# KKKSQJ/DeepLearning

Hardware: NVIDIA H100
Metric: images/sec (ResNet-50 training step) (higher is better)
Workload: dtype bf16

## Files before the change

deeplearning_b200/csrc/abi_conv.cu:

```cuda
#include <string.h>
#include "../../include/b200cls.h"
#include "conv_gemm.cuh"
#include "conv1x1_stream.cuh"
#include "conv_tap64.cuh"
#include "host_utils.h"
#include "wgrad_gemm.cuh"

using namespace b200;

namespace {

constexpr uint32_t kFwdDescLbo = 16, kFwdDescSbo = 1024;
constexpr uint32_t kWgDescLbo = 8192, kWgDescSbo = 1024, kWgDescKstep = 2048;

struct Box3 {
  int b1, b2, b3;
};

Box3 choose_box(long long d1, long long d2, long long d3, int P) {
  Box3 best{P, 1, 1};
  double best_cost = -1;
  for (int b1 = 1; b1 <= P; b1 <<= 1) {
    for (int b2 = 1; b1 * b2 <= P; b2 <<= 1) {
      const int b3 = P / (b1 * b2);
// ... 101 lines not shown
  for (int q = 0; q < 4; ++q) o1[q] = o2[q] = o3[q] = 0;
  if (bx.b3 >= 4) {
    *qb = Box3{bx.b1, bx.b2, bx.b3 / 4};
    for (int q = 0; q < 4; ++q) o3[q] = q * (bx.b3 / 4);
  } else if (bx.b3 == 2) {
    *qb = Box3{bx.b1, bx.b2 / 2, 1};
    if (bx.b2 >= 2) {
      for (int q = 0; q < 4; ++q) {
        o2[q] = (q & 1) * (bx.b2 / 2);
        o3[q] = q >> 1;
      }
    } else {
      *qb = Box3{bx.b1 / 2, 1, 1};
      for (int q = 0; q < 4; ++q) {
        o1[q] = (q & 1) * (bx.b1 / 2);
        o3[q] = q >> 1;
      }
    }
  } else if (bx.b2 >= 4) {
    *qb = Box3{bx.b1, bx.b2 / 4, 1};
    for (int q = 0; q < 4; ++q) o2[q] = q * (bx.b2 / 4);
  } else if (bx.b2 == 2) {
    *qb = Box3{bx.b1 / 2, 1, 1};
    for (int q = 0; q < 4; ++q) {
      o1[q] = (q & 1) * (bx.b1 / 2);
      o2[q] = q >> 1;
    }
  } else {
    *qb = Box3{bx.b1 / 4, 1, 1};
    for (int q = 0; q < 4; ++q) o1[q] = q * (bx.b1 / 4);
  }
}

int setup_output(ConvGemmParams& p, const View& dv, int N, int out_f32, const View* auxv) {
  const long long d1 = dv.dims[1], d2 = dv.dims[2], d3 = dv.dims[3];
  const Box3 bx = choose_box(d1, d2, d3, 128);
  p.box1 = bx.b1, p.box2 = bx.b2, p.box3 = bx.b3;
  p.dim1 = static_cast<int>(d1), p.dim2 = static_cast<int>(d2), p.dim3 = static_cast<int>(d3);
  p.tiles1 = static_cast<int>((d1 + bx.b1 - 1) / bx.b1);
  p.tiles2 = static_cast<int>((d2 + bx.b2 - 1) / bx.b2);
  p.tiles3 = static_cast<int>((d3 + bx.b3 - 1) / bx.b3);
  p.N = N;
  const int BN = N <= 64 ? 64 : 128;
  p.n_tiles = (N + BN - 1) / BN;
  Box3 qb;
  quarter_box(bx, &qb, p.qoff1, p.qoff2, p.qoff3);
  p.out_f32 = out_f32;
  if (dv.base != nullptr) {
    uint32_t box[4] = {out_f32 ? 32u : 64u, (uint32_t)qb.b1, (uint32_t)qb.b2, (uint32_t)qb.b3};
    int rc = out_f32 ? encode_tmap_f32(&p.d_map, dv.base, 4, dv.dims, dv.strides, box)
                     : encode_tmap_bf16(&p.d_map, dv.base, 4, dv.dims, dv.strides, box);
    if (rc) return rc;
  }
  p.has_aux_out = 0;
  if (auxv != nullptr) {
    uint32_t box[4] = {64u, (uint32_t)qb.b1, (uint32_t)qb.b2, (uint32_t)qb.b3};
    int rc = encode_tmap_bf16(&p.aux_map, auxv->base, 4, auxv->dims, auxv->strides, box);
    if (rc) return rc;
    p.has_aux_out = 1;
  }
  return OK;
}
Box3 box_of(const ConvGemmParams& p) { return Box3{p.box1, p.box2, p.box3}; }

bool bn_mask_complete(const b200_bn_mask_t* m) { return m->x_raw && m->scale && m->shift && m->stats; }
void set_bn_mask(ConvGemmParams& p, const b200_bn_mask_t* m, const View& dv) {
  p.mask_in = static_cast<const __nv_bfloat16*>(m->x_raw);
  p.ms1 = static_cast<long long>(dv.strides[1]);
  p.ms2 = static_cast<long long>(dv.strides[2]);
// ... 29 lines not shown
  if (p.residual) f |= p.res_f32 ? kEpiResF32 : kEpiResBf16;
  if (p.has_aux_out) f |= kEpiAux;
  if (p.out_f32) f |= kEpiOutF32;
  if (p.out_direct) f |= kEpiDirect;
  if (p.stats) f |= kEpiStats;
  if (p.rowscale) f |= kEpiRowscale;
  if (p.affine) f = (f & ~(kEpiBias | kEpiColscale)) | kEpiAffine;
  if (p.mask_in) f |= p.bn_scale ? kEpiBnMask : kEpiMask;
  if (p.bn_scale) f &= ~kEpiStats;
  return f;
}

#define B200_EPI_LIST(X)                                                                                  \
  X(kEpiStats)                                              \
  X(0)                                                      \
  X(kEpiResBf16)                                            \
  X(kEpiBias)                                               \
  X(kEpiBias | kEpiResF32 | kEpiOutF32)                     \
  X(kEpiBias | kEpiColscale | kEpiResF32 | kEpiOutF32)      \
  X(kEpiBias | (2 << kEpiActShift) | kEpiAux)               \
  X(3 << kEpiActShift)                                      \
  X((3 << kEpiActShift) | kEpiStats)                        \
  X(kEpiOutF32)                                             \
  X(kEpiBias | kEpiOutF32)                                  \
  X(kEpiAffine | kEpiResBf16 | (1 << kEpiActShift))        \
  X(kEpiAffine | (1 << kEpiActShift))                      \
  X(kEpiAffine)                                            \
  X(kEpiMask | kEpiResBf16 | kEpiStats)                    \
  X(kEpiBnMask)                                            \
  X(kEpiBnMask | kEpiBias)                                 \
  X(kEpiBias | (1 << kEpiActShift))                        \
  X(kEpiBias | kEpiStats)

bool tap64_ok(const ConvGemmParams& p) {
  const int f = epilogue_flags(p);
  return p.N == 64 && p.n_tiles == 1 && p.k_per_tap == 64 && p.k_blocks_per_tap == 1 && !p.var_taps && !p.chan_window &&
         p.num_taps >= 2 && p.num_taps <= 9 && (f == 0 || f == kEpiStats) && p.dim1 % p.box1 == 0 && p.dim2 % p.box2 == 0 &&
         p.dim3 % p.box3 == 0;
}
template <bool kStats>
int launch_tap64(const ConvGemmParams& q, int grid, cudaStream_t st) {
  static bool configured = false;
  if (!configured) {
    B200_CHECK_CUDA(cudaFuncSetAttribute(conv_tap64_kernel<kStats>, cudaFuncAttributeMaxDynamicSharedMemorySize, kTap64SmemBytes));
    configured = true;
  }
  B200_CHECK_CUDA(launch_pdl(conv_tap64_kernel<kStats>, dim3(grid), dim3(384), kTap64SmemBytes, st, q));
  B200_LAUNCHED();
  return OK;
}

template <int BLOCK_N>
int launch_conv_gemm(const ConvGemmParams& p, cudaStream_t st) {
  const int tiles = p.tiles1 * p.tiles2 * p.tiles3 * p.n_tiles;
  const int grid = conv_grid(tiles, p.n_tiles, p.stats != nullptr);
  B200_REQUIRE(grid > 0, "conv_gemm: %d channel blocks exceed the SM count (BN statistics need grid %% n_tiles == 0)", p.n_tiles);
  ConvGemmParams q = p;
  q.desc_lbo = kFwdDescLbo;
  q.desc_sbo = kFwdDescSbo;
  if constexpr (BLOCK_N == 64) {
    if (tap64_ok(p)) return p.stats != nullptr ? launch_tap64<true>(q, grid, st) : launch_tap64<false>(q, grid, st);
  }
  switch (epilogue_flags(p)) {
#define B200_EPI_CASE(F) \
  case (F):              \
    return launch_conv_gemm_epi<BLOCK_N, (F)>(q, grid, st);
    B200_EPI_LIST(B200_EPI_CASE)
#undef B200_EPI_CASE
    default:
      return launch_conv_gemm_epi<BLOCK_N, kEpiGeneric>(q, grid, st);
  }
}


bool stream_ok(long long pixels, int K, int N) {
  return (K == 64 || K == 128 || K == 256) && N % 256 == 0 && pixels % 128 == 0 && pixels / 128 < (1LL << 30);
}
int stream_grid(long long pixels, int N) {
  const int n_tiles = N / 256;
  const long long items = pixels / 128 * n_tiles;
  int grid = items < device_sm_count() ? static_cast<int>(items) : device_sm_count();
  return grid / n_tiles * n_tiles;
}

template <int KB, int MODE>
int launch_stream(const StreamParams& q, int grid, cudaStream_t st) {
  using Cfg = StreamCfg<KB, MODE>;
  static bool configured = false;
  if (!configured) {
    B200_CHECK_CUDA(cudaFuncSetAttribute(conv1x1_stream_kernel<KB, MODE>, cudaFuncAttributeMaxDynamicSharedMemorySize,
                                         Cfg::SMEM_BYTES));
    configured = true;
  }
// ... 188 lines not shown
static int fwd_stats_rows(int B, int H, int W, int Cout, int ksize, int stride, int BN) {
  const Dims3 d = out_dims(B, H, W, ksize, stride);
  const Box3 bx = choose_box(d.d1, d.d2, d.d3, 128);
  const long long m_tiles = ((d.d1 + bx.b1 - 1) / bx.b1) * ((d.d2 + bx.b2 - 1) / bx.b2) * ((d.d3 + bx.b3 - 1) / bx.b3);
  const int n_tiles = (Cout + BN - 1) / BN;
  const long long tiles = m_tiles * n_tiles;
  const int grid = conv_grid(tiles > (1 << 30) ? (1 << 30) : static_cast<int>(tiles), n_tiles, true);
  return grid / n_tiles * (BN == 64 ? 8 : 4);
}

int b200_conv2d_fwd_stats_rows(int B, int H, int W, int Cout, int ksize, int stride) {
  return fwd_stats_rows(B, H, W, Cout, ksize, stride, block_n_for(Cout));
}

static int conv_fwd(const void* x, const void* w, void* y, int B, int H, int W, int Cin, int Cout, int ksize, int stride,
                    float* stats, const float* bias, int act, const void* residual, float* out_f32, long long ld_out,
                    const float* bn_scale, const float* bn_shift, int y_f32, int Cg, void* stream) {
  B200_REQUIRE(ksize == 1 || ksize == 3 || (ksize == 2 && stride == 2), "conv2d_fwd: ksize %d / stride %d unsupported", ksize, stride);
  B200_REQUIRE(stride == 1 || stride == 2, "conv2d_fwd: stride %d unsupported (1 or 2)", stride);
  B200_REQUIRE(Cin % 8 == 0 && Cout % 8 == 0, "conv2d_fwd: Cin=%d / Cout=%d must be multiples of 8", Cin, Cout);
  B200_REQUIRE(B > 0 && H > 0 && W > 0, "conv2d_fwd: empty input");
  B200_REQUIRE(stride == 1 || (H >= 2 && W >= 2), "conv2d_fwd: stride-2 needs H,W >= 2");
  B200_REQUIRE(out_f32 == nullptr || (ksize == 1 && stride == 1), "conv2d_fwd: fp32 output only for 1x1/s1");
  B200_REQUIRE((bn_scale == nullptr) == (bn_shift == nullptr), "conv2d_fwd: bn_scale and bn_shift go together");
  B200_REQUIRE(bn_scale == nullptr || (Cout % 64 == 0 && bias == nullptr && stats == nullptr && out_f32 == nullptr && act <= 1 && !y_f32),
               "conv2d_fwd + folded BN: Cout=%d must be a multiple of 64, no bias / statistics / fp32 output", Cout);
  cudaStream_t st = static_cast<cudaStream_t>(stream);
  const int Ho = out_dim(H, ksize, stride), Wo = out_dim(W, ksize, stride);
  ConvGemmParams p;
  memset(&p, 0, sizeof(p));
  int rc;
  View dv = act_view(y, B, Ho, Wo, Cout, ksize == 1 && stride == 1);
  if (out_f32 != nullptr) dv.base = nullptr;
  if ((rc = setup_output(p, dv, Cout, y_f32, nullptr))) return rc;
  const int BN = Cg ? 64 : block_n_for(Cout);
  p.n_tiles = (Cout + BN - 1) / BN;
  p.chan_window = Cg ? 1 : 0;
  p.k_per_tap = Cg ? 64 : Cin;
  p.k_blocks_per_tap = Cg ? 1 : (Cin + 63) / 64;
  p.num_taps = ksize * ksize;
  if ((rc = encode_taps(p, p.a_maps, x, B, H, W, Cin, ksize, stride, box_of(p)))) return rc;
  for (int t = 0; t < p.num_taps; ++t) p.tap_w[t] = static_cast<int8_t>(t);
  if ((rc = encode_matrix(&p.b_map, w, static_cast<long long>(p.num_taps) * p.k_per_tap, Cout, BN))) return rc;
  p.stats = stats;
  p.bias = bias;
  p.act = act;
  p.residual = residual;
  p.rs1 = static_cast<long long>(dv.strides[1]);
  p.rs2 = static_cast<long long>(dv.strides[2]);
  p.rs3 = static_cast<long long>(dv.strides[3]);
  p.out_direct = out_f32;
  p.ld_out = ld_out;
  if (bn_scale != nullptr) {
    p.affine = 1;
    p.colscale = bn_scale;
    p.bias = bn_shift;
  }
  return Cg ? launch_conv_gemm<64>(p, st) : dispatch_conv_gemm(p, Cout, st);
}

int b200_conv2d_fwd(const void* x, const void* w, void* y, int B, int H, int W, int Cin, int Cout, int ksize, int stride,
                    float* stats, const float* bias, int act, const void* residual, float* out_f32, long long ld_out,
                    const float* bn_scale, const float* bn_shift, void* stream) {
  return conv_fwd(x, w, y, B, H, W, Cin, Cout, ksize, stride, stats, bias, act, residual, out_f32, ld_out, bn_scale, bn_shift,
                  0, 0, stream);
}

int b200_conv2d_fwd_f32(const void* x, const void* w, float* y, int B, int H, int W, int Cin, int Cout, int ksize,
                        int stride, const float* bias, void* stream) {
  return conv_fwd(x, w, y, B, H, W, Cin, Cout, ksize, stride, nullptr, bias, 0, nullptr, nullptr, 0, nullptr, nullptr, 1, 0,
                  stream);
}

static int conv_dgrad(const void* dy, const void* wd, void* dx, int B, int H, int W, int Cin, int Cout, int ksize,
                      int stride, const void* residual, const b200_bn_mask_t* bn_mask, int Cg, void* stream) {
  B200_REQUIRE(ksize == 1 || ksize == 3 || (ksize == 2 && stride == 2), "conv2d_dgrad: ksize %d / stride %d unsupported", ksize, stride);
  B200_REQUIRE(stride == 1 || stride == 2, "conv2d_dgrad: stride %d unsupported", stride);
  B200_REQUIRE(Cin % 8 == 0 && Cout % 8 == 0, "conv2d_dgrad: Cin=%d / Cout=%d must be multiples of 8", Cin, Cout);
  B200_REQUIRE(bn_mask == nullptr || (stride == 1 && Cin % 64 == 0 && bn_mask_complete(bn_mask)),
               "conv2d_dgrad: the fused BatchNorm-backward reduce needs stride 1, Cin %% 64 == 0 and every bn_mask field "
               "(Cin=%d, stride=%d)", Cin, stride);
  cudaStream_t st = static_cast<cudaStream_t>(stream);
  const int Ho = out_dim(H, ksize, stride), Wo = out_dim(W, ksize, stride);
  const bool flat = (ksize == 1 && stride == 1);
  const int BN = Cg ? 64 : block_n_for(Cin);
  const int k_per_tap = Cg ? 64 : Cout;
  int rc;
  CUtensorMap b_map;
  if ((rc = encode_matrix(&b_map, wd, static_cast<long long>(ksize * ksize) * k_per_tap, Cin, BN))) return rc;
  const int nphase = (stride == 2 && ksize >= 2) ? 2 : 1;
  for (int ph = 0; ph < nphase; ++ph) {
    for (int pw = 0; pw < nphase; ++pw) {
      ConvGemmParams p;
      memset(&p, 0, sizeof(p));
      p.b_map = b_map;
      View dv = flat ? make_flat_view(dx, static_cast<long long>(B) * H * W, Cin)
                     : make_view(dx, B, H, W, Cin, stride, ph, pw);
      if ((rc = setup_output(p, dv, Cin, 0, nullptr))) return rc;
      p.n_tiles = (Cin + BN - 1) / BN;
      p.chan_window = Cg ? 1 : 0;
      p.k_per_tap = k_per_tap;
      p.k_blocks_per_tap = Cg ? 1 : (Cout + 63) / 64;
      if ((rc = encode_view(&p.a_maps[0], act_view(dy, B, Ho, Wo, Cout, flat), box_of(p)))) return rc;
      for (int i = 1; i < 4; ++i) p.a_maps[i] = p.a_maps[0];
      int nt = 0;
      if (ksize == 1) {
        p.tap_map[0] = 0, p.tap_o1[0] = 0, p.tap_o2[0] = 0, p.tap_w[0] = 0;
        nt = 1;
      } else if (stride == 1) {
        for (int kh = 0; kh < 3; ++kh)
          for (int kw = 0; kw < 3; ++kw) {
            p.tap_map[nt] = 0;
            p.tap_o1[nt] = static_cast<int8_t>(1 - kw);
            p.tap_o2[nt] = static_cast<int8_t>(1 - kh);
            p.tap_w[nt] = static_cast<int8_t>(kh * 3 + kw);
            ++nt;
          }
      } else if (ksize == 2) {
        p.tap_map[0] = 0, p.tap_o1[0] = 0, p.tap_o2[0] = 0;
        p.tap_w[0] = static_cast<int8_t>(ph * 2 + pw);
        nt = 1;
      } else {
        for (int kh = 0; kh < 3; ++kh) {
          if (((ph + 1 - kh) & 1) != 0) continue;
          for (int kw = 0; kw < 3; ++kw) {
            if (((pw + 1 - kw) & 1) != 0) continue;
            p.tap_map[nt] = 0;
            p.tap_o1[nt] = static_cast<int8_t>((pw + 1 - kw) / 2);
            p.tap_o2[nt] = static_cast<int8_t>((ph + 1 - kh) / 2);
            p.tap_w[nt] = static_cast<int8_t>(kh * 3 + kw);
            ++nt;
          }
        }
      }
      p.num_taps = nt;
      if (residual != nullptr) {
// ... 323 lines not shown
```

deeplearning_b200/csrc/common.cuh:

```cuda
#pragma once
#include <cuda_runtime.h>
#include <cuda_bf16.h>
#include <cuda.h>
#include <stdint.h>
#include "wgmma.cuh"

namespace b200 {

constexpr int kNumSMs = 132;

__device__ __forceinline__ void pdl_wait() { asm volatile("griddepcontrol.wait;" ::: "memory"); }

__device__ __forceinline__ uint32_t smem_u32(const void* p) {
  return static_cast<uint32_t>(__cvta_generic_to_shared(p));
}

__device__ __forceinline__ bool elect_one() {
  uint32_t pred = 0;
  asm volatile(
      "{\n\t.reg .pred P;\n\t"
      "elect.sync _|P, 0xffffffff;\n\t"
      "selp.b32 %0, 1, 0, P;\n\t}\n"
      : "=r"(pred));
  return pred != 0;
// ... 16 lines not shown
  uint32_t addr = smem_u32(bar);
  asm volatile(
      "{\n\t.reg .pred P1;\n\t"
      "WAIT_%=:\n\t"
      "mbarrier.try_wait.parity.shared::cta.b64 P1, [%0], %1;\n\t"
      "@P1 bra DONE_%=;\n\t"
      "bra WAIT_%=;\n\t"
      "DONE_%=:\n\t}\n" ::"r"(addr),
      "r"(parity)
      : "memory");
}

__device__ __forceinline__ void mbar_wait_backoff(uint64_t* bar, uint32_t parity) {
  uint32_t addr = smem_u32(bar);
  asm volatile(
      "{\n\t.reg .pred P1;\n\t"
      "WAIT_%=:\n\t"
      "mbarrier.try_wait.parity.shared::cta.b64 P1, [%0], %1;\n\t"
      "@P1 bra DONE_%=;\n\t"
      "nanosleep.u32 40;\n\t"
      "bra WAIT_%=;\n\t"
      "DONE_%=:\n\t}\n" ::"r"(addr),
      "r"(parity)
      : "memory");
}

__device__ __forceinline__ void sts128(uint32_t addr, uint32_t a, uint32_t b, uint32_t c, uint32_t d) {
  asm volatile("st.shared.v4.b32 [%0], {%1, %2, %3, %4};" ::"r"(addr), "r"(a), "r"(b), "r"(c), "r"(d) : "memory");
}
__device__ __forceinline__ uint32_t lds32(uint32_t addr) {
  uint32_t v;
  asm volatile("ld.shared.b32 %0, [%1];" : "=r"(v) : "r"(addr) : "memory");
  return v;
}
__device__ __forceinline__ uint64_t f2_pack(float lo, float hi) {
  uint64_t r;
  asm("mov.b64 %0, {%1, %2};" : "=l"(r) : "f"(lo), "f"(hi));
  return r;
}
__device__ __forceinline__ void f2_unpack(uint64_t v, float& lo, float& hi) {
  asm("mov.b64 {%0, %1}, %2;" : "=f"(lo), "=f"(hi) : "l"(v));
}
__device__ __forceinline__ uint64_t f2_add(uint64_t a, uint64_t b) {
  float a0, a1, b0, b1;
  f2_unpack(a, a0, a1);
  f2_unpack(b, b0, b1);
  return f2_pack(__fadd_rn(a0, b0), __fadd_rn(a1, b1));
}
__device__ __forceinline__ uint64_t f2_mul(uint64_t a, uint64_t b) {
  float a0, a1, b0, b1;
  f2_unpack(a, a0, a1);
  f2_unpack(b, b0, b1);
  return f2_pack(__fmul_rn(a0, b0), __fmul_rn(a1, b1));
}
__device__ __forceinline__ uint64_t f2_bcast(float c) { return f2_pack(c, c); }
__device__ __forceinline__ uint64_t f2_fma(uint64_t a, uint64_t b, uint64_t c) {
  float a0, a1, b0, b1, c0, c1;
  f2_unpack(a, a0, a1);
  f2_unpack(b, b0, b1);
  f2_unpack(c, c0, c1);
  return f2_pack(__fmaf_rn(a0, b0, c0), __fmaf_rn(a1, b1, c1));
}

__device__ __forceinline__ void fence_proxy_async_smem() {
  asm volatile("fence.proxy.async.shared::cta;" ::: "memory");
}
// ... 146 lines not shown
```

deeplearning_b200/csrc/conv_gemm.cuh:

```cuda
#pragma once
#include <cstdio>
#include "common.cuh"

namespace b200 {

constexpr int kMaxTaps = 16;

struct alignas(64) ConvGemmParams {
  CUtensorMap a_maps[4];
  CUtensorMap b_map;
  CUtensorMap d_map;
  CUtensorMap aux_map;
  int num_taps;
  int k_per_tap;
  int k_blocks_per_tap;
  int tiles1, tiles2, tiles3;
  int box1, box2, box3;
  int dim1, dim2, dim3;
  int qoff1[4], qoff2[4], qoff3[4];
  int n_tiles;
  int N;
  int8_t tap_map[kMaxTaps];
  int8_t tap_o1[kMaxTaps];
  int8_t tap_o2[kMaxTaps];
  int8_t tap_w[kMaxTaps];
  float* stats;
  const float* bias;
  const float* colscale;
  int act;
  int out_f32;
  int res_f32;
  int has_aux_out;
  const void* residual;
  long long rs1, rs2, rs3;
  const __nv_bfloat16* aux_in;
  long long as1, as2, as3;
  uint32_t desc_lbo, desc_sbo;
  float* out_direct;
  long long ld_out;
  const float* rowscale;
  int rows_per_sample;
  int var_taps;
  int kb_total;
  int16_t tap_kb[kMaxTaps];
  int32_t tap_k0[kMaxTaps];
  const __nv_bfloat16* mask_in;
  long long ms1, ms2, ms3;
  int affine;
  const float* bn_scale;
  const float* bn_shift;
  int chan_window;
};

template <int BLOCK_N>
struct ConvGemmCfg {
  static constexpr int BLOCK_M = 128;
  static constexpr int BLOCK_K = 64;
  static constexpr int A_BYTES = BLOCK_M * BLOCK_K * 2;
  static constexpr int B_BYTES = BLOCK_N * BLOCK_K * 2;
  static constexpr int STAGES = BLOCK_N == 128 ? 4 : 5;
  static constexpr int STAGE_BYTES = A_BYTES + B_BYTES;
  static constexpr int EPI_WARPS = 4;
  static constexpr int SLAB_BYTES = 32 * 128;
  static constexpr int STAGING_BYTES = EPI_WARPS * 2 * SLAB_BYTES;
  static constexpr int IMG_BYTES = BLOCK_M * BLOCK_N * 4;
  static constexpr int IMGS = BLOCK_N == 128 ? 1 : 2;
  static constexpr int BAR_BYTES = 256;
  static constexpr int SMEM_BYTES = STAGES * STAGE_BYTES + STAGING_BYTES + IMGS * IMG_BYTES + BAR_BYTES + 1024;
  static constexpr int THREADS = 512;
  static_assert(SMEM_BYTES <= 227 * 1024, "shared memory of one H100 block");
  static_assert(2 * STAGES + 2 * IMGS <= BAR_BYTES / 8, "mbarriers");
};

__device__ __forceinline__ void gelu_parts(float x, float& tail, float& e) {
  const float az = fabsf(x) * 0.70710678118654752f;
  float t;
  asm("rcp.approx.ftz.f32 %0, %1;" : "=f"(t) : "f"(fmaf(0.3275911f, az, 1.0f)));
  float poly = fmaf(1.061405429f, t, -1.453152027f);
  poly = fmaf(poly, t, 1.421413741f);
  poly = fmaf(poly, t, -0.284496736f);
  poly = fmaf(poly, t, 0.254829592f);
  asm("ex2.approx.ftz.f32 %0, %1;" : "=f"(e) : "f"(-1.4426950408889634f * az * az));
  tail = 0.5f * poly * t * e;
}
__device__ __forceinline__ float gelu_erf(float x) {
  float tail, e;
  gelu_parts(x, tail, e);
  return x * (x >= 0.f ? 1.0f - tail : tail);
}
__device__ __forceinline__ float gelu_erf_grad(float x) {
  float tail, e;
  gelu_parts(x, tail, e);
  const float cdf = x >= 0.f ? 1.0f - tail : tail;
  return fmaf(x * 0.3989422804014327f, e, cdf);
}

__device__ __forceinline__ void gelu_parts2(float x0, float x1, uint64_t& cdf, uint64_t& e) {
  const uint64_t az = f2_pack(fabsf(x0) * 0.70710678118654752f, fabsf(x1) * 0.70710678118654752f);
  float d0, d1, t0, t1, g0, g1, e0, e1, h0, h1;
  f2_unpack(f2_fma(f2_bcast(0.3275911f), az, f2_bcast(1.0f)), d0, d1);
  asm("rcp.approx.ftz.f32 %0, %1;" : "=f"(t0) : "f"(d0));
  asm("rcp.approx.ftz.f32 %0, %1;" : "=f"(t1) : "f"(d1));
  const uint64_t t = f2_pack(t0, t1);
  uint64_t poly = f2_fma(f2_bcast(1.061405429f), t, f2_bcast(-1.453152027f));
// ... 15 lines not shown
__device__ __forceinline__ void gelu_erf_val_grad2(float& x0, float& x1, float& g0, float& g1) {
  uint64_t cdf, e;
  gelu_parts2(x0, x1, cdf, e);
  const uint64_t x = f2_pack(x0, x1);
  f2_unpack(f2_fma(f2_mul(x, f2_bcast(0.3989422804014327f)), e, cdf), g0, g1);
  f2_unpack(f2_mul(x, cdf), x0, x1);
}

#ifdef CONV_PROFILE
#define CPROF_DECL(N) long long cp_t[N] = {}; long long cp_0 = clock64(), cp_1;
#define CPROF_TICK(i) { cp_1 = clock64(); cp_t[i] += cp_1 - cp_0; cp_0 = cp_1; }
#else
#define CPROF_DECL(N)
#define CPROF_TICK(i)
#endif

template <int S>
__device__ __forceinline__ void butterfly_step(float (&px)[32], int lane) {
  const bool up = (lane & S) != 0;
#pragma unroll
  for (int i = 0; i < S; ++i) {
    const float send = up ? px[i] : px[i + S];
    const float keep = up ? px[i + S] : px[i];
    px[i] = keep + __shfl_xor_sync(0xffffffffu, send, S);
  }
}

constexpr int kEpiGeneric = -1;
constexpr int kEpiBias = 1, kEpiColscale = 2, kEpiActShift = 2 , kEpiResBf16 = 16, kEpiResF32 = 32,
              kEpiAux = 64, kEpiOutF32 = 128, kEpiDirect = 256, kEpiStats = 512,
              kEpiRowscale = 1024 ,
              kEpiAffine = 2048, kEpiMask = 4096, kEpiBnMask = 8192;

template <int BLOCK_N, int EPI = kEpiGeneric>
__global__ void __launch_bounds__(512, 1) conv_gemm_kernel(const __grid_constant__ ConvGemmParams p) {
  static_assert(BLOCK_N == 64 || BLOCK_N == 128, "64- or 128-column tiles");
  using Cfg = ConvGemmCfg<BLOCK_N>;
  constexpr int STAGES = Cfg::STAGES;
  constexpr int IMGS = Cfg::IMGS;
  extern __shared__ uint8_t smem_raw[];
  uint8_t* smem = reinterpret_cast<uint8_t*>((reinterpret_cast<uintptr_t>(smem_raw) + 1023) & ~uintptr_t(1023));
  uint8_t* stage_base = smem;
  uint8_t* staging = smem + STAGES * Cfg::STAGE_BYTES;
  uint8_t* img = staging + Cfg::STAGING_BYTES;
  uint64_t* bars = reinterpret_cast<uint64_t*>(img + IMGS * Cfg::IMG_BYTES);
  uint64_t* full_bar = bars;
  uint64_t* empty_bar = bars + STAGES;
  uint64_t* img_full = bars + 2 * STAGES;
  uint64_t* img_empty = bars + 2 * STAGES + IMGS;

  const int warp_idx = threadIdx.x >> 5;
  const int lane = threadIdx.x & 31;
  const int m_tiles = p.tiles1 * p.tiles2 * p.tiles3;
  const int num_tiles = m_tiles * p.n_tiles;
  const int num_kb = p.var_taps ? p.kb_total : p.num_taps * p.k_blocks_per_tap;

  if (warp_idx == 0 && lane == 0) {
    for (int i = 0; i < 4; ++i) tma_prefetch_desc(&p.a_maps[i]);
    tma_prefetch_desc(&p.b_map);
    tma_prefetch_desc(&p.d_map);
    for (int i = 0; i < STAGES; ++i) {
      mbar_init(&full_bar[i], 1);
      mbar_init(&empty_bar[i], 2);
    }
    for (int i = 0; i < IMGS; ++i) {
      mbar_init(&img_full[i], 8);
      mbar_init(&img_empty[i], Cfg::EPI_WARPS);
    }
    fence_mbar_init();
  }
  __syncthreads();
  pdl_wait();

  if (warp_idx < 4) {
    setmaxnreg_dec<40>();
    if (warp_idx == 0 && lane == 0) {
      int stage = 0;
      uint32_t phase = 0;
      CPROF_DECL(2)
      for (int tile = blockIdx.x; tile < num_tiles; tile += gridDim.x) {
        const int n_tile = tile % p.n_tiles;
        const int m_tile = tile / p.n_tiles;
        const int t1 = m_tile % p.tiles1;
        const int t2 = (m_tile / p.tiles1) % p.tiles2;
        const int t3 = m_tile / (p.tiles1 * p.tiles2);
        const int c1 = t1 * p.box1, c2 = t2 * p.box2, c3 = t3 * p.box3;
        int tap = 0, cb = 0;
        int kb_in_tap = p.var_taps ? p.tap_kb[0] : p.k_blocks_per_tap;
        for (int kb = 0; kb < num_kb; ++kb, ++cb) {
          if (cb == kb_in_tap) {
            cb = 0;
            ++tap;
            if (p.var_taps) kb_in_tap = p.tap_kb[tap];
          }
          const int wk = p.var_taps ? p.tap_k0[tap] + cb * 64 : p.tap_w[tap] * p.k_per_tap + cb * 64;
          CPROF_TICK(1)
          mbar_wait_backoff(&empty_bar[stage], phase ^ 1);
          CPROF_TICK(0)
          uint8_t* a_dst = stage_base + stage * Cfg::STAGE_BYTES;
          uint8_t* b_dst = a_dst + Cfg::A_BYTES;
          mbar_expect_tx(&full_bar[stage], Cfg::STAGE_BYTES);
          tma_load_4d(a_dst, &p.a_maps[p.tap_map[tap]], &full_bar[stage], p.chan_window ? n_tile * BLOCK_N : cb * 64, c1 + p.tap_o1[tap],
                      c2 + p.tap_o2[tap], c3);
          tma_load_2d(b_dst, &p.b_map, &full_bar[stage], wk, n_tile * BLOCK_N);
          if (++stage == STAGES) {
            stage = 0;
            phase ^= 1;
          }
        }
      }
#ifdef CONV_PROFILE
      if (blockIdx.x == 0) {
        const int nt = (num_tiles - 1) / gridDim.x + 1;
        printf("conv producer: wait_empty %lld issue %lld  (cycles/tile, %d tiles, %d k-blocks)\n", cp_t[0] / nt, cp_t[1] / nt, nt, num_kb);
      }
#endif
    }
  } else if (warp_idx < 12) {
    setmaxnreg_dec<112>();
    const int wg = (warp_idx - 4) >> 2;
    const uint64_t desc_a0 = make_smem_desc_sw128(smem_u32(stage_base) + wg * 8192, p.desc_lbo, p.desc_sbo);
    const uint64_t desc_b0 = make_smem_desc_sw128(smem_u32(stage_base) + Cfg::A_BYTES, p.desc_lbo, p.desc_sbo);
    int stage = 0;
    uint32_t phase = 0;
    int it = 0;
    CPROF_DECL(3)
    for (int tile = blockIdx.x; tile < num_tiles; tile += gridDim.x, ++it) {
      float acc[BLOCK_N / 2];
#pragma unroll
      for (int i = 0; i < BLOCK_N / 2; ++i) acc[i] = 0.f;
      int prev = -1;
      CPROF_TICK(2)
      for (int kb = 0; kb < num_kb; ++kb) {
        mbar_wait(&full_bar[stage], phase);
        wgmma_fence();
        const uint64_t soff = static_cast<uint64_t>(stage) * (Cfg::STAGE_BYTES >> 4);
        const uint64_t da = desc_a0 + soff, db = desc_b0 + soff;
#pragma unroll
        for (int k = 0; k < 4; ++k) Wgmma<BLOCK_N, 0, 0>::mma(acc, da + 2 * k, db + 2 * k, 1u);
        wgmma_commit();
        wgmma_wait<1>();
        if (prev >= 0 && (threadIdx.x & 127) == 0) mbar_arrive(&empty_bar[prev]);
        prev = stage;
        if (++stage == STAGES) {
          stage = 0;
          phase ^= 1;
        }
      }
      wgmma_wait<0>();
      wgmma_reg_fence(acc);
      if ((threadIdx.x & 127) == 0) mbar_arrive(&empty_bar[prev]);
      CPROF_TICK(0)
      const int b = IMGS == 1 ? 0 : it % IMGS;
      mbar_wait(&img_empty[b], ((it / IMGS) & 1) ^ 1);
      CPROF_TICK(1)
      acc_to_img<BLOCK_N>(acc, smem_u32(img + b * Cfg::IMG_BYTES), BLOCK_N, 64 * wg, 0);
      __syncwarp();
      if (lane == 0) mbar_arrive(&img_full[b]);
    }
#ifdef CONV_PROFILE
    if (blockIdx.x == 0 && lane == 0 && (warp_idx & 3) == 0) {
      const int nt = (num_tiles - 1) / gridDim.x + 1;
      printf("conv mma wg %d: main loop %lld wait img_empty %lld acc->img %lld  (cycles/tile)\n", wg, cp_t[0] / nt, cp_t[1] / nt,
             cp_t[2] / nt);
    }
#endif
  } else {
    setmaxnreg_inc<248>();
    const int q = warp_idx - 12;
    const int row = q * 32 + lane;
    const uint32_t stage_s = smem_u32(staging + q * 2 * Cfg::SLAB_BYTES);
    const uint32_t row_s = lane * 128;
    const uint32_t sw = (lane & 7) << 4;
    uint32_t stat_off[8];
#pragma unroll
    for (int m = 0; m < 8; ++m) stat_off[m] = m * 128 + ((((lane >> 2) ^ m) << 4) | ((lane & 3) << 2));
    constexpr bool G = EPI < 0;
    constexpr bool kAffine = !G && (EPI & kEpiAffine) != 0;
    constexpr bool kBnMask = !G && (EPI & kEpiBnMask) != 0;
    constexpr bool kMask = !G && (EPI & (kEpiMask | kEpiBnMask)) != 0;
    const int N = p.N;
    const float* const bias = (!kAffine && (G || (EPI & kEpiBias))) ? p.bias : nullptr;
    const float* const colscale = (!kAffine && (G || (EPI & kEpiColscale))) ? p.colscale : nullptr;
    const int act_bits = G ? p.act : ((EPI >> kEpiActShift) & 3);
// ... 379 lines not shown
```

deeplearning_b200/csrc/wgmma.cuh:

```cuda
#pragma once
#include <stdint.h>

namespace b200 {

template <int N, int TA, int TB>
struct Wgmma;

template <int TA, int TB>
struct Wgmma<16, TA, TB> {
  static __device__ __forceinline__ void mma(float (&d)[8], uint64_t da, uint64_t db, uint32_t accumulate) {
    asm volatile(
        "{\n.reg .pred p;\n"
        "setp.ne.b32 p, %10, 0;\n"
        "wgmma.mma_async.sync.aligned.m64n16k16.f32.bf16.bf16 "
        "{%0, %1, %2, %3, %4, %5, %6, %7}, "
        "%8, %9, p, 1, 1, %11, %12;\n}\n"
        : "+f"(d[0]), "+f"(d[1]), "+f"(d[2]), "+f"(d[3]), "+f"(d[4]), "+f"(d[5]), "+f"(d[6]), "+f"(d[7])
        : "l"(da), "l"(db), "r"(accumulate), "n"(TA), "n"(TB));
  }
};

template <int TA, int TB>
struct Wgmma<32, TA, TB> {
  static __device__ __forceinline__ void mma(float (&d)[16], uint64_t da, uint64_t db, uint32_t accumulate) {
// ... 125 lines not shown
    asm volatile(
        "{\n.reg .pred p;\n"
        "setp.ne.b32 p, %130, 0;\n"
        "wgmma.mma_async.sync.aligned.m64n256k16.f32.bf16.bf16 "
        "{%0, %1, %2, %3, %4, %5, %6, %7, %8, %9, %10, %11, %12, %13, %14, %15, "
        "%16, %17, %18, %19, %20, %21, %22, %23, %24, %25, %26, %27, %28, %29, %30, %31, "
        "%32, %33, %34, %35, %36, %37, %38, %39, %40, %41, %42, %43, %44, %45, %46, %47, "
        "%48, %49, %50, %51, %52, %53, %54, %55, %56, %57, %58, %59, %60, %61, %62, %63, "
        "%64, %65, %66, %67, %68, %69, %70, %71, %72, %73, %74, %75, %76, %77, %78, %79, "
        "%80, %81, %82, %83, %84, %85, %86, %87, %88, %89, %90, %91, %92, %93, %94, %95, "
        "%96, %97, %98, %99, %100, %101, %102, %103, %104, %105, %106, %107, %108, %109, %110, %111, "
        "%112, %113, %114, %115, %116, %117, %118, %119, %120, %121, %122, %123, %124, %125, %126, %127}, "
        "%128, %129, p, 1, 1, %131, %132;\n}\n"
        : "+f"(d[0]), "+f"(d[1]), "+f"(d[2]), "+f"(d[3]), "+f"(d[4]), "+f"(d[5]), "+f"(d[6]), "+f"(d[7]),
          "+f"(d[8]), "+f"(d[9]), "+f"(d[10]), "+f"(d[11]), "+f"(d[12]), "+f"(d[13]), "+f"(d[14]), "+f"(d[15]),
          "+f"(d[16]), "+f"(d[17]), "+f"(d[18]), "+f"(d[19]), "+f"(d[20]), "+f"(d[21]), "+f"(d[22]), "+f"(d[23]),
          "+f"(d[24]), "+f"(d[25]), "+f"(d[26]), "+f"(d[27]), "+f"(d[28]), "+f"(d[29]), "+f"(d[30]), "+f"(d[31]),
          "+f"(d[32]), "+f"(d[33]), "+f"(d[34]), "+f"(d[35]), "+f"(d[36]), "+f"(d[37]), "+f"(d[38]), "+f"(d[39]),
          "+f"(d[40]), "+f"(d[41]), "+f"(d[42]), "+f"(d[43]), "+f"(d[44]), "+f"(d[45]), "+f"(d[46]), "+f"(d[47]),
          "+f"(d[48]), "+f"(d[49]), "+f"(d[50]), "+f"(d[51]), "+f"(d[52]), "+f"(d[53]), "+f"(d[54]), "+f"(d[55]),
          "+f"(d[56]), "+f"(d[57]), "+f"(d[58]), "+f"(d[59]), "+f"(d[60]), "+f"(d[61]), "+f"(d[62]), "+f"(d[63]),
          "+f"(d[64]), "+f"(d[65]), "+f"(d[66]), "+f"(d[67]), "+f"(d[68]), "+f"(d[69]), "+f"(d[70]), "+f"(d[71]),
          "+f"(d[72]), "+f"(d[73]), "+f"(d[74]), "+f"(d[75]), "+f"(d[76]), "+f"(d[77]), "+f"(d[78]), "+f"(d[79]),
          "+f"(d[80]), "+f"(d[81]), "+f"(d[82]), "+f"(d[83]), "+f"(d[84]), "+f"(d[85]), "+f"(d[86]), "+f"(d[87]),
          "+f"(d[88]), "+f"(d[89]), "+f"(d[90]), "+f"(d[91]), "+f"(d[92]), "+f"(d[93]), "+f"(d[94]), "+f"(d[95]),
          "+f"(d[96]), "+f"(d[97]), "+f"(d[98]), "+f"(d[99]), "+f"(d[100]), "+f"(d[101]), "+f"(d[102]), "+f"(d[103]),
          "+f"(d[104]), "+f"(d[105]), "+f"(d[106]), "+f"(d[107]), "+f"(d[108]), "+f"(d[109]), "+f"(d[110]), "+f"(d[111]),
          "+f"(d[112]), "+f"(d[113]), "+f"(d[114]), "+f"(d[115]), "+f"(d[116]), "+f"(d[117]), "+f"(d[118]), "+f"(d[119]),
          "+f"(d[120]), "+f"(d[121]), "+f"(d[122]), "+f"(d[123]), "+f"(d[124]), "+f"(d[125]), "+f"(d[126]), "+f"(d[127])
        : "l"(da), "l"(db), "r"(accumulate), "n"(TA), "n"(TB));
  }
};

}
```

Before: 8699.

## Add halo-tile 3x3 conv path with resident weights and register-A WGMMA

```diff
diff --git a/deeplearning_b200/csrc/abi_conv.cu b/deeplearning_b200/csrc/abi_conv.cu
--- a/deeplearning_b200/csrc/abi_conv.cu
+++ b/deeplearning_b200/csrc/abi_conv.cu
@@ -157,9 +157,9 @@
   }
 }
 
-int setup_output(ConvGemmParams& p, const View& dv, int N, int out_f32, const View* auxv) {
+int setup_output(ConvGemmParams& p, const View& dv, int N, int out_f32, const View* auxv, const Box3* force_box = nullptr) {
   const long long d1 = dv.dims[1], d2 = dv.dims[2], d3 = dv.dims[3];
-  const Box3 bx = choose_box(d1, d2, d3, 128);
+  const Box3 bx = force_box != nullptr ? *force_box : choose_box(d1, d2, d3, 128);
   p.box1 = bx.b1, p.box2 = bx.b2, p.box3 = bx.b3;
   p.dim1 = static_cast<int>(d1), p.dim2 = static_cast<int>(d2), p.dim3 = static_cast<int>(d3);
   p.tiles1 = static_cast<int>((d1 + bx.b1 - 1) / bx.b1);
@@ -255,10 +255,29 @@
   X(kEpiBias | (1 << kEpiActShift))                        \
   X(kEpiBias | kEpiStats)
 
+constexpr Box3 kHaloTile{8, 8, 2};
+constexpr Box3 kHaloBox{8 + 2, 8 + 2, 2};
+bool halo_shape_ok(int B, int H, int W, int Cin, int Cout, int ksize, int stride, int Cg) {
+  return ksize == 3 && stride == 1 && Cin == 64 && Cout == 64 && Cg == 0 && H % 8 == 0 && W % 8 == 0 && B % 2 == 0;
+}
+template <int EPI>
+int launch_halo(const ConvGemmParams& q, int grid, cudaStream_t st) {
+  using Cfg = ConvGemmCfg<64, true>;
+  static bool configured = false;
+  if (!configured) {
+    B200_CHECK_CUDA(cudaFuncSetAttribute(conv_gemm_kernel<64, EPI, true>, cudaFuncAttributeMaxDynamicSharedMemorySize,
+                                         Cfg::SMEM_BYTES));
+    configured = true;
+  }
+  B200_CHECK_CUDA(launch_pdl(conv_gemm_kernel<64, EPI, true>, dim3(grid), dim3(Cfg::THREADS), Cfg::SMEM_BYTES, st, q));
+  B200_LAUNCHED();
+  return OK;
+}
+
 bool tap64_ok(const ConvGemmParams& p) {
   const int f = epilogue_flags(p);
   return p.N == 64 && p.n_tiles == 1 && p.k_per_tap == 64 && p.k_blocks_per_tap == 1 && !p.var_taps && !p.chan_window &&
-         p.num_taps >= 2 && p.num_taps <= 9 && (f == 0 || f == kEpiStats) && p.dim1 % p.box1 == 0 && p.dim2 % p.box2 == 0 &&
+         p.num_taps == 4 && (f == 0 || f == kEpiStats) && p.dim1 % p.box1 == 0 && p.dim2 % p.box2 == 0 &&
          p.dim3 % p.box3 == 0;
 }
 template <bool kStats>
@@ -282,6 +301,15 @@
   q.desc_lbo = kFwdDescLbo;
   q.desc_sbo = kFwdDescSbo;
   if constexpr (BLOCK_N == 64) {
+    if (p.halo) {
+      const int f = epilogue_flags(p);
+      B200_REQUIRE(p.num_taps == 9 && p.k_per_tap == 64 && p.N == 64 && p.box1 == 8 && p.box2 == 8 && p.box3 == 2,
+                   "conv_gemm: halo launch of an unsupported geometry");
+      if (f == 0) return launch_halo<0>(q, grid, st);
+      if (f == kEpiStats) return launch_halo<kEpiStats>(q, grid, st);
+      if (f == kEpiBnMask) return launch_halo<kEpiBnMask>(q, grid, st);
+      B200_REQUIRE(false, "conv_gemm: halo launch with unsupported epilogue flags %d", f);
+    }
     if (tap64_ok(p)) return p.stats != nullptr ? launch_tap64<true>(q, grid, st) : launch_tap64<false>(q, grid, st);
   }
   switch (epilogue_flags(p)) {
@@ -536,14 +564,17 @@
   int rc;
   View dv = act_view(y, B, Ho, Wo, Cout, ksize == 1 && stride == 1);
   if (out_f32 != nullptr) dv.base = nullptr;
-  if ((rc = setup_output(p, dv, Cout, y_f32, nullptr))) return rc;
+  const bool halo = halo_shape_ok(B, H, W, Cin, Cout, ksize, stride, Cg) && bias == nullptr && act == 0 &&
+                    residual == nullptr && out_f32 == nullptr && bn_scale == nullptr && !y_f32;
+  p.halo = halo ? 1 : 0;
+  if ((rc = setup_output(p, dv, Cout, y_f32, nullptr, halo ? &kHaloTile : nullptr))) return rc;
   const int BN = Cg ? 64 : block_n_for(Cout);
   p.n_tiles = (Cout + BN - 1) / BN;
   p.chan_window = Cg ? 1 : 0;
   p.k_per_tap = Cg ? 64 : Cin;
   p.k_blocks_per_tap = Cg ? 1 : (Cin + 63) / 64;
   p.num_taps = ksize * ksize;
-  if ((rc = encode_taps(p, p.a_maps, x, B, H, W, Cin, ksize, stride, box_of(p)))) return rc;
+  if ((rc = encode_taps(p, p.a_maps, x, B, H, W, Cin, ksize, stride, halo ? kHaloBox : box_of(p)))) return rc;
   for (int t = 0; t < p.num_taps; ++t) p.tap_w[t] = static_cast<int8_t>(t);
   if ((rc = encode_matrix(&p.b_map, w, static_cast<long long>(p.num_taps) * p.k_per_tap, Cout, BN))) return rc;
   p.stats = stats;
@@ -592,6 +623,7 @@
   int rc;
   CUtensorMap b_map;
   if ((rc = encode_matrix(&b_map, wd, static_cast<long long>(ksize * ksize) * k_per_tap, Cin, BN))) return rc;
+  const bool halo = halo_shape_ok(B, H, W, Cin, Cout, ksize, stride, Cg) && residual == nullptr;
   const int nphase = (stride == 2 && ksize >= 2) ? 2 : 1;
   for (int ph = 0; ph < nphase; ++ph) {
     for (int pw = 0; pw < nphase; ++pw) {
@@ -600,12 +632,13 @@
       p.b_map = b_map;
       View dv = flat ? make_flat_view(dx, static_cast<long long>(B) * H * W, Cin)
                      : make_view(dx, B, H, W, Cin, stride, ph, pw);
-      if ((rc = setup_output(p, dv, Cin, 0, nullptr))) return rc;
+      p.halo = halo ? 1 : 0;
+      if ((rc = setup_output(p, dv, Cin, 0, nullptr, halo ? &kHaloTile : nullptr))) return rc;
       p.n_tiles = (Cin + BN - 1) / BN;
       p.chan_window = Cg ? 1 : 0;
       p.k_per_tap = k_per_tap;
       p.k_blocks_per_tap = Cg ? 1 : (Cout + 63) / 64;
-      if ((rc = encode_view(&p.a_maps[0], act_view(dy, B, Ho, Wo, Cout, flat), box_of(p)))) return rc;
+      if ((rc = encode_view(&p.a_maps[0], act_view(dy, B, Ho, Wo, Cout, flat), halo ? kHaloBox : box_of(p)))) return rc;
       for (int i = 1; i < 4; ++i) p.a_maps[i] = p.a_maps[0];
       int nt = 0;
       if (ksize == 1) {
diff --git a/deeplearning_b200/csrc/common.cuh b/deeplearning_b200/csrc/common.cuh
--- a/deeplearning_b200/csrc/common.cuh
+++ b/deeplearning_b200/csrc/common.cuh
@@ -72,6 +72,12 @@
   uint32_t v;
   asm volatile("ld.shared.b32 %0, [%1];" : "=r"(v) : "r"(addr) : "memory");
   return v;
+}
+__device__ __forceinline__ void ldsm_x4(uint32_t addr, uint32_t (&a)[4]) {
+  asm volatile("ldmatrix.sync.aligned.m8n8.x4.shared.b16 {%0, %1, %2, %3}, [%4];"
+               : "=r"(a[0]), "=r"(a[1]), "=r"(a[2]), "=r"(a[3])
+               : "r"(addr)
+               : "memory");
 }
 __device__ __forceinline__ uint64_t f2_pack(float lo, float hi) {
   uint64_t r;
diff --git a/deeplearning_b200/csrc/conv_gemm.cuh b/deeplearning_b200/csrc/conv_gemm.cuh
--- a/deeplearning_b200/csrc/conv_gemm.cuh
+++ b/deeplearning_b200/csrc/conv_gemm.cuh
@@ -50,9 +50,15 @@
   const float* bn_scale;
   const float* bn_shift;
   int chan_window;
+  int halo;
 };
 
-template <int BLOCK_N>
+constexpr int kHaloW = 10;
+constexpr int kHaloBytes = 2 * kHaloW * kHaloW * 128;
+constexpr int kHaloStages = 2;
+constexpr int kHaloWeightBytes = 9 * 64 * 128;
+
+template <int BLOCK_N, bool HALO = false>
 struct ConvGemmCfg {
   static constexpr int BLOCK_M = 128;
   static constexpr int BLOCK_K = 64;
@@ -66,10 +72,12 @@
   static constexpr int IMG_BYTES = BLOCK_M * BLOCK_N * 4;
   static constexpr int IMGS = BLOCK_N == 128 ? 1 : 2;
   static constexpr int BAR_BYTES = 256;
-  static constexpr int SMEM_BYTES = STAGES * STAGE_BYTES + STAGING_BYTES + IMGS * IMG_BYTES + BAR_BYTES + 1024;
+  static constexpr int RING_BYTES = HALO ? kHaloWeightBytes + kHaloStages * kHaloBytes : STAGES * STAGE_BYTES;
+  static constexpr int SMEM_BYTES = RING_BYTES + STAGING_BYTES + IMGS * IMG_BYTES + BAR_BYTES + 1024;
   static constexpr int THREADS = 512;
   static_assert(SMEM_BYTES <= 227 * 1024, "shared memory of one H100 block");
-  static_assert(2 * STAGES + 2 * IMGS <= BAR_BYTES / 8, "mbarriers");
+  static_assert(2 * STAGES + 2 * IMGS + 1 <= BAR_BYTES / 8, "mbarriers");
+  static_assert(!HALO || (BLOCK_N == 64 && kHaloStages <= STAGES), "halo mode: 64-column tiles");
 };
 
 __device__ __forceinline__ void gelu_parts(float x, float& tail, float& e) {
@@ -151,22 +159,24 @@
               kEpiRowscale = 1024 ,
               kEpiAffine = 2048, kEpiMask = 4096, kEpiBnMask = 8192;
 
-template <int BLOCK_N, int EPI = kEpiGeneric>
+template <int BLOCK_N, int EPI = kEpiGeneric, bool HALO = false>
 __global__ void __launch_bounds__(512, 1) conv_gemm_kernel(const __grid_constant__ ConvGemmParams p) {
   static_assert(BLOCK_N == 64 || BLOCK_N == 128, "64- or 128-column tiles");
-  using Cfg = ConvGemmCfg<BLOCK_N>;
+  using Cfg = ConvGemmCfg<BLOCK_N, HALO>;
   constexpr int STAGES = Cfg::STAGES;
   constexpr int IMGS = Cfg::IMGS;
   extern __shared__ uint8_t smem_raw[];
   uint8_t* smem = reinterpret_cast<uint8_t*>((reinterpret_cast<uintptr_t>(smem_raw) + 1023) & ~uintptr_t(1023));
   uint8_t* stage_base = smem;
-  uint8_t* staging = smem + STAGES * Cfg::STAGE_BYTES;
+  uint8_t* staging = smem + Cfg::RING_BYTES;
   uint8_t* img = staging + Cfg::STAGING_BYTES;
   uint64_t* bars = reinterpret_cast<uint64_t*>(img + IMGS * Cfg::IMG_BYTES);
   uint64_t* full_bar = bars;
   uint64_t* empty_bar = bars + STAGES;
   uint64_t* img_full = bars + 2 * STAGES;
   uint64_t* img_empty = bars + 2 * STAGES + IMGS;
+  uint64_t* w_full = bars + 2 * STAGES + 2 * IMGS;
+  uint8_t* halo_base = stage_base + kHaloWeightBytes;
 
   const int warp_idx = threadIdx.x >> 5;
   const int lane = threadIdx.x & 31;
@@ -180,8 +190,9 @@
     tma_prefetch_desc(&p.d_map);
     for (int i = 0; i < STAGES; ++i) {
       mbar_init(&full_bar[i], 1);
-      mbar_init(&empty_bar[i], 2);
+      mbar_init(&empty_bar[i], HALO ? 8 : 2);
     }
+    if (HALO) mbar_init(w_full, 1);
     for (int i = 0; i < IMGS; ++i) {
       mbar_init(&img_full[i], 8);
       mbar_init(&img_empty[i], Cfg::EPI_WARPS);
@@ -193,7 +204,25 @@
 
   if (warp_idx < 4) {
     setmaxnreg_dec<40>();
-    if (warp_idx == 0 && lane == 0) {
+    if (HALO && warp_idx == 0 && lane == 0) {
+      mbar_expect_tx(w_full, kHaloWeightBytes);
+      for (int t = 0; t < 9; ++t) tma_load_2d(stage_base + t * 8192, &p.b_map, w_full, p.tap_w[t] * p.k_per_tap, 0);
+      int stage = 0;
+      uint32_t phase = 0;
+      for (int tile = blockIdx.x; tile < num_tiles; tile += gridDim.x) {
+        const int t1 = tile % p.tiles1;
+        const int t2 = (tile / p.tiles1) % p.tiles2;
+        const int t3 = tile / (p.tiles1 * p.tiles2);
+        mbar_wait_backoff(&empty_bar[stage], phase ^ 1);
+        mbar_expect_tx(&full_bar[stage], kHaloBytes);
+        tma_load_4d(halo_base + stage * kHaloBytes, &p.a_maps[0], &full_bar[stage], 0, t1 * p.box1 - 1, t2 * p.box2 - 1,
+                    t3 * p.box3);
+        if (++stage == kHaloStages) {
+          stage = 0;
+          phase ^= 1;
+        }
+      }
+    } else if (!HALO && warp_idx == 0 && lane == 0) {
       int stage = 0;
       uint32_t phase = 0;
       CPROF_DECL(2)
@@ -240,6 +269,10 @@
     const int wg = (warp_idx - 4) >> 2;
     const uint64_t desc_a0 = make_smem_desc_sw128(smem_u32(stage_base) + wg * 8192, p.desc_lbo, p.desc_sbo);
     const uint64_t desc_b0 = make_smem_desc_sw128(smem_u32(stage_base) + Cfg::A_BYTES, p.desc_lbo, p.desc_sbo);
+    const int hrow0 = (wg * kHaloW + 2 * (warp_idx & 3) + ((lane >> 3) & 1)) * kHaloW + (lane & 7);
+    const uint32_t hcol = static_cast<uint32_t>(lane >> 4);
+    const uint64_t desc_w0 = make_smem_desc_sw128(smem_u32(stage_base), p.desc_lbo, p.desc_sbo);
+    if (HALO) mbar_wait(w_full, 0);
     int stage = 0;
     uint32_t phase = 0;
     int it = 0;
@@ -248,27 +281,63 @@
       float acc[BLOCK_N / 2];
 #pragma unroll
       for (int i = 0; i < BLOCK_N / 2; ++i) acc[i] = 0.f;
-      int prev = -1;
       CPROF_TICK(2)
-      for (int kb = 0; kb < num_kb; ++kb) {
+      if constexpr (HALO) {
         mbar_wait(&full_bar[stage], phase);
-        wgmma_fence();
-        const uint64_t soff = static_cast<uint64_t>(stage) * (Cfg::STAGE_BYTES >> 4);
-        const uint64_t da = desc_a0 + soff, db = desc_b0 + soff;
-#pragma unroll
-        for (int k = 0; k < 4; ++k) Wgmma<BLOCK_N, 0, 0>::mma(acc, da + 2 * k, db + 2 * k, 1u);
-        wgmma_commit();
-        wgmma_wait<1>();
-        if (prev >= 0 && (threadIdx.x & 127) == 0) mbar_arrive(&empty_bar[prev]);
-        prev = stage;
-        if (++stage == STAGES) {
+        const uint32_t hs = smem_u32(halo_base + stage * kHaloBytes);
+        auto tap_row = [&](int t) { return hrow0 + (p.tap_o2[t] + 1) * kHaloW + p.tap_o1[t] + 1; };
+        uint32_t frag[2][4];
+        int row = tap_row(0);
+        ldsm_x4(hs + row * 128 + ((hcol ^ (row & 7)) << 4), frag[0]);
+#pragma unroll 1
+        for (int t = 0; t < 9; ++t) {
+          const uint32_t rs = hs + row * 128, rsw = row & 7;
+          const int next = t + 1 < 9 ? tap_row(t + 1) : row;
+#pragma unroll
+          for (int k = 0; k < 4; ++k) {
+            wgmma_fence();
+            WgmmaRegA<64, 0>::mma(acc, frag[k & 1], desc_w0 + static_cast<uint64_t>(t) * (8192 >> 4) + 2 * k, 1u);
+            wgmma_commit();
+            if (k < 3) {
+              wgmma_wait<1>();
+              ldsm_x4(rs + (((2 * (k + 1) + hcol) ^ rsw) << 4), frag[(k + 1) & 1]);
+            } else if (t + 1 < 9) {
+              wgmma_wait<1>();
+              ldsm_x4(hs + next * 128 + ((hcol ^ (next & 7)) << 4), frag[0]);
+            }
+          }
+          row = next;
+        }
+        __syncwarp();
+        if (lane == 0) mbar_arrive(&empty_bar[stage]);
+        if (++stage == kHaloStages) {
           stage = 0;
           phase ^= 1;
         }
+        wgmma_wait<0>();
+        wgmma_reg_fence(acc);
+      } else {
+        int prev = -1;
+        for (int kb = 0; kb < num_kb; ++kb) {
+          mbar_wait(&full_bar[stage], phase);
+          wgmma_fence();
+          const uint64_t soff = static_cast<uint64_t>(stage) * (Cfg::STAGE_BYTES >> 4);
+          const uint64_t da = desc_a0 + soff, db = desc_b0 + soff;
+#pragma unroll
+          for (int k = 0; k < 4; ++k) Wgmma<BLOCK_N, 0, 0>::mma(acc, da + 2 * k, db + 2 * k, 1u);
+          wgmma_commit();
+          wgmma_wait<1>();
+          if (prev >= 0 && (threadIdx.x & 127) == 0) mbar_arrive(&empty_bar[prev]);
+          prev = stage;
+          if (++stage == STAGES) {
+            stage = 0;
+            phase ^= 1;
+          }
+        }
+        wgmma_wait<0>();
+        wgmma_reg_fence(acc);
+        if ((threadIdx.x & 127) == 0) mbar_arrive(&empty_bar[prev]);
       }
-      wgmma_wait<0>();
-      wgmma_reg_fence(acc);
-      if ((threadIdx.x & 127) == 0) mbar_arrive(&empty_bar[prev]);
       CPROF_TICK(0)
       const int b = IMGS == 1 ? 0 : it % IMGS;
       mbar_wait(&img_empty[b], ((it / IMGS) & 1) ^ 1);
diff --git a/deeplearning_b200/csrc/wgmma.cuh b/deeplearning_b200/csrc/wgmma.cuh
--- a/deeplearning_b200/csrc/wgmma.cuh
+++ b/deeplearning_b200/csrc/wgmma.cuh
@@ -181,4 +181,25 @@
   }
 };
 
+template <int N, int TB>
+struct WgmmaRegA;
+
+template <int TB>
+struct WgmmaRegA<64, TB> {
+  static __device__ __forceinline__ void mma(float (&d)[32], const uint32_t (&a)[4], uint64_t db, uint32_t accumulate) {
+    asm volatile(
+        "{\n.reg .pred p;\n"
+        "setp.ne.b32 p, %37, 0;\n"
+        "wgmma.mma_async.sync.aligned.m64n64k16.f32.bf16.bf16 "
+        "{%0, %1, %2, %3, %4, %5, %6, %7, %8, %9, %10, %11, %12, %13, %14, %15, "
+        "%16, %17, %18, %19, %20, %21, %22, %23, %24, %25, %26, %27, %28, %29, %30, %31}, "
+        "{%32, %33, %34, %35}, %36, p, 1, 1, %38;\n}\n"
+        : "+f"(d[0]), "+f"(d[1]), "+f"(d[2]), "+f"(d[3]), "+f"(d[4]), "+f"(d[5]), "+f"(d[6]), "+f"(d[7]),
+          "+f"(d[8]), "+f"(d[9]), "+f"(d[10]), "+f"(d[11]), "+f"(d[12]), "+f"(d[13]), "+f"(d[14]), "+f"(d[15]),
+          "+f"(d[16]), "+f"(d[17]), "+f"(d[18]), "+f"(d[19]), "+f"(d[20]), "+f"(d[21]), "+f"(d[22]), "+f"(d[23]),
+          "+f"(d[24]), "+f"(d[25]), "+f"(d[26]), "+f"(d[27]), "+f"(d[28]), "+f"(d[29]), "+f"(d[30]), "+f"(d[31])
+        : "r"(a[0]), "r"(a[1]), "r"(a[2]), "r"(a[3]), "l"(db), "r"(accumulate), "n"(TB));
+  }
+};
+
 }
```

Result: no change. 8764, median of 6 (+0.8%).
